# aalto-speech/AaltoASR

Measured on AMD Instinct MI355X. Metric: frames/sec GMM log-lik (39-d, 50k Gauss) + MFCC, 1/2/4/8 MI355X, higher is better.
Workload: dtype f32 (2-term fp16 split on the matrix cores, f32 accumulate); 1 GPU; configs[2]: full MFCC chain (FFT -> mel -> log -> DCT -> delta/delta-delta, CMS, normalisation) + 50000-Gaussian scoring + 2-byte LNA codes on 1 h of synthetic 16 kHz audio as 360 x 10 s utterances (449280 frames), int16 samples resident in HBM; dim=39, gaussians=50000, states=3125, gpus_flag=1

## Files before the change

aaltoasr_amd/csrc/lna_device.h:

```cpp
#pragma once
#include <hip/hip_runtime.h>

#include <cmath>
#include <cstdint>

namespace aasr {

#define LN2_D 0.69314718055994530942
#define LOG_TINY_D (-115.12925464970228420090)
#define LN_FLT_MIN_F (-87.33654475f)

__device__ __forceinline__ double float_cast_loglik(float ll) {
  if (ll >= LN_FLT_MIN_F) return (double)ll;
  if (ll < -103.98f) return -INFINITY;
  const float L1 = 1.44269502162933349609375f;
  const float L2 = 1.92596303350001e-08f;
  const float hi = ll * L1;
  const float lo = fmaf(ll, L1, -hi) + ll * L2;
  const float t = __builtin_amdgcn_exp2f(hi + 149.0f) * (1.0f + lo * 0.69314718f);
  const float q = rintf(t);
  if (q <= 0.0f) return -INFINITY;
  return (double)(__builtin_amdgcn_logf(q) * 0.69314718f) - 149.0 * LN2_D;
}

template <class T>
__device__ __forceinline__ T wave_reduce_max(T v) {
  for (int o = 32; o > 0; o >>= 1) {
    T u = __shfl_xor(v, o, 64);
    v = u > v ? u : v;
  }
  return v;
}
__device__ __forceinline__ double wave_reduce_sum(double v) {
  for (int o = 32; o > 0; o >>= 1) v += __shfl_xor(v, o, 64);
  return v;
}

__device__ __forceinline__ void lna_store(float lp, int lnabytes, int64_t o,
                                          float *__restrict__ lp_out,
                                          uint8_t *__restrict__ bytes_out) {
  if (lp_out) lp_out[o] = lp;
  if (bytes_out) {
    if (lnabytes == 4) {
      ((float *)bytes_out)[o] = lp;
    } else {
      unsigned short code;
      if (lp < -36.008f) {
        code = 0xffff;
      } else {
        int temp = (int)(-1820.0 * (double)lp + .5);
        unsigned b0 = (temp >> 8) & 255, b1 = temp & 255;
        code = (unsigned short)(b0 | (b1 << 8));
      }
      ((unsigned short *)bytes_out)[o] = code;
    }
  }
}

__device__ __forceinline__ float cast_f(float ll) {
  return ll >= LN_FLT_MIN_F ? ll : (float)float_cast_loglik(ll);
}


template <int VPT, int JSAFE = 0>
__device__ __forceinline__ void lna_row_from_registers(const float (&v)[VPT], int S, int tid, int wave, int lane,
                                                       double *red, int normalize, int lnabytes, int64_t f,
                                                       bool store, float *__restrict__ lp_out,
                                                       uint8_t *__restrict__ bytes_out) {
  double logz = 0.0;
  if (lnabytes == 2 && !lp_out) {
    float mr = -INFINITY;
#pragma unroll
    for (int j = 0; j < VPT; j++) mr = fmaxf(mr, v[j]);
    mr = wave_reduce_max(mr);
    if (lane == 0) red[wave] = (double)mr;
    __syncthreads();
    mr = (float)fmax(fmax(red[0], red[1]), fmax(red[2], red[3]));
    __syncthreads();
    if (mr >= -51.0f) {
      double z = 0.0;
      if (normalize) {
#pragma unroll
        for (int j = 0; j < VPT; j++) z += (double)__builtin_amdgcn_exp2f((v[j] - mr) * 1.44269504088896340736f);
      }
      z = wave_reduce_sum(z);
      if (lane == 0) red[4 + wave] = z;
      __syncthreads();
      z = (red[4] + red[5]) + (red[6] + red[7]);
      __syncthreads();
      if (normalize) logz = (double)mr + log(z);
      if (!store) return;
#pragma unroll
      for (int j = 0; j < VPT; j++) {
        const int i = tid + 256 * j;
        if (j < JSAFE || i < S) {
          const float lp = fmaxf((float)((double)v[j] - logz), (float)LOG_TINY_D);
          lna_store(lp, 2, f * (int64_t)S + i, nullptr, bytes_out);
        }
      }
      return;
    }
  }
  if (normalize) {
    float m = -INFINITY;
#pragma unroll
    for (int j = 0; j < VPT; j++) m = fmaxf(m, cast_f(v[j]));
    m = wave_reduce_max(m);
    if (lane == 0) red[wave] = (double)m;
    __syncthreads();
    m = (float)fmax(fmax(red[0], red[1]), fmax(red[2], red[3]));
    __syncthreads();
    double z = 0.0;
    if (m > -INFINITY) {
#pragma unroll
      for (int j = 0; j < VPT; j++)
        z += (double)__builtin_amdgcn_exp2f((cast_f(v[j]) - m) * 1.44269504088896340736f);
    }
    z = wave_reduce_sum(z);
    if (lane == 0) red[4 + wave] = z;
    __syncthreads();
    z = (red[4] + red[5]) + (red[6] + red[7]);
    __syncthreads();
    if (m > -INFINITY) logz = (double)m + log(z);
  }
  if (!store) return;
#pragma unroll
  for (int j = 0; j < VPT; j++) {
    const int i = tid + 256 * j;
    if (j < JSAFE || i < S) {
      const double vd = v[j] >= LN_FLT_MIN_F ? (double)v[j] : float_cast_loglik(v[j]);
      const float lp = fmaxf((float)(vd - logz), (float)LOG_TINY_D);
      lna_store(lp, lnabytes, f * (int64_t)S + i, lp_out, bytes_out);
    }
  }
}

}
```

aaltoasr_amd/csrc/lna_encode.hip:

```cpp
#include <hip/hip_runtime.h>

#include <algorithm>
#include <cmath>
#include <cstdlib>

#include "common.h"
#include "lna_device.h"

namespace aasr {

__global__ __launch_bounds__(256) void k_state_norm_lna(
    const float *__restrict__ loglik, int64_t F, int S, int64_t in_pitch, int normalize,
    int lnabytes, float *__restrict__ lp_out, uint8_t *__restrict__ bytes_out) {
  __shared__ double red[8];
  const int tid = threadIdx.x, wave = tid >> 6, lane = tid & 63;
  for (int64_t f = blockIdx.x; f < F; f += gridDim.x) {
    const float *row = loglik + f * in_pitch;
    double logz = 0.0;
    if (normalize) {
      double m = -INFINITY;
      for (int i = tid; i < S; i += 256) {
        double v = float_cast_loglik(row[i]);
        m = v > m ? v : m;
      }
      m = wave_reduce_max(m);
      if (lane == 0) red[wave] = m;
      __syncthreads();
      m = fmax(fmax(red[0], red[1]), fmax(red[2], red[3]));
      __syncthreads();
      if (m > -INFINITY) {
        double z = 0.0;
        for (int i = tid; i < S; i += 256) {
          double v = float_cast_loglik(row[i]);
          z += (double)expf((float)(v - m));
        }
        z = wave_reduce_sum(z);
        if (lane == 0) red[4 + wave] = z;
        __syncthreads();
        z = (red[4] + red[5]) + (red[6] + red[7]);
        __syncthreads();
        logz = m + log(z);
      }
    }
    for (int i = tid; i < S; i += 256) {
      double v = float_cast_loglik(row[i]);
      double lpd = v - logz;
      if (!(lpd >= LOG_TINY_D)) lpd = LOG_TINY_D;
      float lp = (float)lpd;
      int64_t o = f * (int64_t)S + i;
      if (lp_out) lp_out[o] = lp;
      if (bytes_out) {
        if (lnabytes == 4) {
          ((float *)bytes_out)[o] = lp;
        } else {
          unsigned short code;
          if ((double)lp < -36.008) {
            code = 0xffff;
          } else {
            int temp = (int)(-1820.0 * (double)lp + .5);
            unsigned b0 = (temp >> 8) & 255, b1 = temp & 255;
            code = (unsigned short)(b0 | (b1 << 8));
          }
          ((unsigned short *)bytes_out)[o] = code;
        }
      }
    }
  }
}


template <int VPT>
__global__ __launch_bounds__(256) void k_state_norm_lna_reg(
    const float *__restrict__ loglik, int64_t F, int S, int64_t in_pitch, int normalize, int lnabytes,
    float *__restrict__ lp_out, uint8_t *__restrict__ bytes_out, const int32_t *__restrict__ colmap) {
  __shared__ double red[8];
  const int tid = threadIdx.x, wave = tid >> 6, lane = tid & 63;
  constexpr int JSAFE = VPT == 4 ? 0 : VPT == 8 ? 4 : VPT == 10 ? 8 : VPT == 13 ? 10 : VPT == 16 ? 13 : 0;
  int col[VPT];
#pragma unroll
  for (int j = 0; j < VPT; j++) {
    const int i = tid + 256 * j;
    col[j] = (colmap && (j < JSAFE || i < S)) ? colmap[i] : i;
  }
  float vn[VPT];
  {
    const float *row = loglik + (int64_t)blockIdx.x * in_pitch;
#pragma unroll
    for (int j = 0; j < VPT; j++) {
      const int i = tid + 256 * j;
      vn[j] = ((j < JSAFE || i < S) && (int64_t)blockIdx.x < F) ? row[col[j]] : -INFINITY;
    }
  }
  for (int64_t f = blockIdx.x; f < F; f += gridDim.x) {
    float v[VPT];
#pragma unroll
    for (int j = 0; j < VPT; j++) v[j] = vn[j];
    if (f + gridDim.x < F) {
      const float *row = loglik + (f + gridDim.x) * in_pitch;
#pragma unroll
      for (int j = 0; j < VPT; j++) {
        const int i = tid + 256 * j;
        vn[j] = (j < JSAFE || i < S) ? row[col[j]] : -INFINITY;
      }
    }
    lna_row_from_registers<VPT, JSAFE>(v, S, tid, wave, lane, red, normalize, lnabytes, f, true, lp_out, bytes_out);
  }
}

__global__ __launch_bounds__(256) void k_state_norm_lna_f64(const double *__restrict__ lik, int64_t F, int S,
                                                            int normalize, int lnabytes, float *__restrict__ lp_out,
                                                            uint8_t *__restrict__ bytes_out) {
  __shared__ double red[4];
  const int tid = threadIdx.x, wave = tid >> 6, lane = tid & 63;
  for (int64_t f = blockIdx.x; f < F; f += gridDim.x) {
    const double *row = lik + f * (int64_t)S;
    double z = 1.0;
    if (normalize) {
      double part = 0.0;
      for (int i = tid; i < S; i += 256) part += (double)(float)row[i];
      part = wave_reduce_sum(part);
      __syncthreads();
      if (lane == 0) red[wave] = part;
      __syncthreads();
      z = (red[0] + red[1]) + (red[2] + red[3]);
      if (z == 0) z = 1.0;
    }
    for (int i = tid; i < S; i += 256) {
      const float o = (float)row[i];
      const double q = (double)o / z;
      const float lp = (float)(q < 1e-50 ? LOG_TINY_D : log(q));
      lna_store(lp, lnabytes, f * (int64_t)S + i, lp_out, bytes_out);
    }
  }
}

void lna_encode_f64_launch(const double *d_lik, int64_t F, int S, int normalize, int lnabytes, float *d_lp,
                           uint8_t *d_bytes, hipStream_t stream) {
  if (F <= 0 || S <= 0) return;
  const int64_t blocks = std::min<int64_t>(F, 8192);
  hipLaunchKernelGGL(k_state_norm_lna_f64, dim3((unsigned)blocks), dim3(256), 0, stream, d_lik, F, S, normalize, lnabytes,
                     d_lp, d_bytes);
  AASR_HIP(hipGetLastError());
}

void lna_encode_launch(const float *d_loglik, int64_t F, int S, int normalize,
                       int lnabytes, float *d_lp, uint8_t *d_bytes, hipStream_t stream, int64_t in_pitch,
                       const int32_t *d_colmap) {
  if (in_pitch <= 0) in_pitch = S;
  if (F <= 0 || S <= 0) return;
  if (d_colmap && S > 256 * 16) raise(AASR_ERR_UNSUPPORTED, "a column map needs the register-resident LNA kernels (S <= 4096)");
  int64_t blocks = F < (1 << 20) ? F : (1 << 20);
  int dev = 0, cus = 256;
  if (hipGetDevice(&dev) == hipSuccess) (void)hipDeviceGetAttribute(&cus, hipDeviceAttributeMultiprocessorCount, dev);
  if (S <= 256 * 16) blocks = std::min<int64_t>(blocks, (int64_t)cus * 32);
  if (S <= 256 * 4)
    hipLaunchKernelGGL(k_state_norm_lna_reg<4>, dim3((unsigned)blocks), dim3(256), 0, stream,
                       d_loglik, F, S, in_pitch, normalize, lnabytes, d_lp, d_bytes, d_colmap);
  else if (S <= 256 * 8)
    hipLaunchKernelGGL(k_state_norm_lna_reg<8>, dim3((unsigned)blocks), dim3(256), 0, stream,
                       d_loglik, F, S, in_pitch, normalize, lnabytes, d_lp, d_bytes, d_colmap);
  else if (S <= 256 * 10)
    hipLaunchKernelGGL(k_state_norm_lna_reg<10>, dim3((unsigned)blocks), dim3(256), 0, stream,
                       d_loglik, F, S, in_pitch, normalize, lnabytes, d_lp, d_bytes, d_colmap);
  else if (S <= 256 * 13)
    hipLaunchKernelGGL(k_state_norm_lna_reg<13>, dim3((unsigned)blocks), dim3(256), 0, stream,
                       d_loglik, F, S, in_pitch, normalize, lnabytes, d_lp, d_bytes, d_colmap);
  else if (S <= 256 * 16)
    hipLaunchKernelGGL(k_state_norm_lna_reg<16>, dim3((unsigned)blocks), dim3(256), 0, stream,
                       d_loglik, F, S, in_pitch, normalize, lnabytes, d_lp, d_bytes, d_colmap);
  else
    hipLaunchKernelGGL(k_state_norm_lna, dim3((unsigned)blocks), dim3(256), 0, stream, d_loglik,
                       F, S, in_pitch, normalize, lnabytes, d_lp, d_bytes);
  AASR_HIP(hipGetLastError());
}

}
```

Before: 43.12 million frames/s.

## Stage grouped LNA 2-byte codes in LDS and write them with wide nontemporal stores

Adds a grouped LNA encoding kernel that normalises G frames per block. It writes each frame's 2-byte codes into an LDS image and then copies the whole group to global memory with 8- or 16-byte nontemporal vector stores. The next row is prefetched with nontemporal loads while the current one is processed. The byte-swap for the code now uses a single perm instruction. The aim is to replace narrow 2-byte global stores with wide coalesced ones, at the cost of extra LDS use, which may lower occupancy, and an extra block-wide barrier per group.

```diff
diff --git a/aaltoasr_amd/csrc/lna_device.h b/aaltoasr_amd/csrc/lna_device.h
--- a/aaltoasr_amd/csrc/lna_device.h
+++ b/aaltoasr_amd/csrc/lna_device.h
@@ -36,6 +36,12 @@
   return v;
 }
 
+__device__ __forceinline__ unsigned lna_code16(float lp) {
+  const int temp = (int)(-1820.0 * (double)lp + .5);
+  const unsigned be = __builtin_amdgcn_perm(0u, (unsigned)temp, 0x0c0c0001u);
+  return lp < -36.008f ? 0xffffu : be;
+}
+
 __device__ __forceinline__ void lna_store(float lp, int lnabytes, int64_t o,
                                           float *__restrict__ lp_out,
                                           uint8_t *__restrict__ bytes_out) {
@@ -44,15 +50,7 @@
     if (lnabytes == 4) {
       ((float *)bytes_out)[o] = lp;
     } else {
-      unsigned short code;
-      if (lp < -36.008f) {
-        code = 0xffff;
-      } else {
-        int temp = (int)(-1820.0 * (double)lp + .5);
-        unsigned b0 = (temp >> 8) & 255, b1 = temp & 255;
-        code = (unsigned short)(b0 | (b1 << 8));
-      }
-      ((unsigned short *)bytes_out)[o] = code;
+      ((unsigned short *)bytes_out)[o] = (unsigned short)lna_code16(lp);
     }
   }
 }
@@ -66,7 +64,8 @@
 __device__ __forceinline__ void lna_row_from_registers(const float (&v)[VPT], int S, int tid, int wave, int lane,
                                                        double *red, int normalize, int lnabytes, int64_t f,
                                                        bool store, float *__restrict__ lp_out,
-                                                       uint8_t *__restrict__ bytes_out) {
+                                                       uint8_t *__restrict__ bytes_out,
+                                                       unsigned short *lds_row = nullptr) {
   double logz = 0.0;
   if (lnabytes == 2 && !lp_out) {
     float mr = -INFINITY;
@@ -95,7 +94,8 @@
         const int i = tid + 256 * j;
         if (j < JSAFE || i < S) {
           const float lp = fmaxf((float)((double)v[j] - logz), (float)LOG_TINY_D);
-          lna_store(lp, 2, f * (int64_t)S + i, nullptr, bytes_out);
+          if (lds_row) lds_row[i] = (unsigned short)lna_code16(lp);
+          else lna_store(lp, 2, f * (int64_t)S + i, nullptr, bytes_out);
         }
       }
       return;
@@ -130,7 +130,8 @@
     if (j < JSAFE || i < S) {
       const double vd = v[j] >= LN_FLT_MIN_F ? (double)v[j] : float_cast_loglik(v[j]);
       const float lp = fmaxf((float)(vd - logz), (float)LOG_TINY_D);
-      lna_store(lp, lnabytes, f * (int64_t)S + i, lp_out, bytes_out);
+      if (lds_row) lds_row[i] = (unsigned short)lna_code16(lp);
+      else lna_store(lp, lnabytes, f * (int64_t)S + i, lp_out, bytes_out);
     }
   }
 }
diff --git a/aaltoasr_amd/csrc/lna_encode.hip b/aaltoasr_amd/csrc/lna_encode.hip
--- a/aaltoasr_amd/csrc/lna_encode.hip
+++ b/aaltoasr_amd/csrc/lna_encode.hip
@@ -3,6 +3,7 @@
 #include <algorithm>
 #include <cmath>
 #include <cstdlib>
+#include <type_traits>
 
 #include "common.h"
 #include "lna_device.h"
@@ -107,6 +108,66 @@
   }
 }
 
+constexpr int kLnaRedBytes = 64;
+template <int VPT, int G>
+__global__ __launch_bounds__(256) void k_state_norm_lna_grp(
+    const float *__restrict__ loglik, int64_t F, int S, int64_t in_pitch, int normalize,
+    uint8_t *__restrict__ bytes_out, const int32_t *__restrict__ colmap) {
+  extern __shared__ __align__(16) unsigned char lna_smem[];
+  double *red = (double *)lna_smem;
+  unsigned char *img = lna_smem + kLnaRedBytes;
+  const int tid = threadIdx.x, wave = tid >> 6, lane = tid & 63;
+  constexpr int JSAFE = VPT == 4 ? 0 : VPT == 8 ? 4 : VPT == 10 ? 8 : VPT == 13 ? 10 : VPT == 16 ? 13 : 0;
+  int col[VPT];
+#pragma unroll
+  for (int j = 0; j < VPT; j++) {
+    const int i = tid + 256 * j;
+    col[j] = (colmap && (j < JSAFE || i < S)) ? colmap[i] : i;
+  }
+  typedef unsigned u32x4 __attribute__((ext_vector_type(4)));
+  typedef unsigned u32x2 __attribute__((ext_vector_type(2)));
+  using vec_t = typename std::conditional<G % 8 == 0, u32x4, u32x2>::type;
+  constexpr int W = (int)sizeof(vec_t);
+  static_assert(G % 4 == 0, "a group's codes must start on an 8-byte boundary at least");
+  const int64_t groups = (F + G - 1) / G;
+  float vn[VPT];
+  {
+    const int64_t f = (int64_t)blockIdx.x * G;
+    const float *row = loglik + f * in_pitch;
+#pragma unroll
+    for (int j = 0; j < VPT; j++) {
+      const int i = tid + 256 * j;
+      vn[j] = ((j < JSAFE || i < S) && f < F) ? row[col[j]] : -INFINITY;
+    }
+  }
+  for (int64_t grp = blockIdx.x; grp < groups; grp += gridDim.x) {
+    const int64_t f0 = grp * G;
+    const int nf = F - f0 < G ? (int)(F - f0) : G;
+    for (int g = 0; g < nf; g++) {
+      float v[VPT];
+#pragma unroll
+      for (int j = 0; j < VPT; j++) v[j] = vn[j];
+      const int64_t fnext = g + 1 < nf ? f0 + g + 1 : (grp + gridDim.x) * G;
+      if (fnext < F) {
+        const float *row = loglik + fnext * in_pitch;
+#pragma unroll
+        for (int j = 0; j < VPT; j++) {
+          const int i = tid + 256 * j;
+          vn[j] = (j < JSAFE || i < S) ? __builtin_nontemporal_load(&row[col[j]]) : -INFINITY;
+        }
+      }
+      lna_row_from_registers<VPT, JSAFE>(v, S, tid, wave, lane, red, normalize, 2, f0 + g, true, nullptr, nullptr,
+                                         (unsigned short *)img + g * S);
+    }
+    __syncthreads();
+    const int nbytes = nf * S * 2;
+    uint8_t *dst = bytes_out + f0 * (int64_t)S * 2;
+    for (int o = tid * W; o + W <= nbytes; o += 256 * W)
+      __builtin_nontemporal_store(*(const vec_t *)(img + o), (vec_t *)(dst + o));
+    for (int o = (nbytes & ~(W - 1)) + tid; o < nbytes; o += 256) dst[o] = img[o];
+  }
+}
+
 __global__ __launch_bounds__(256) void k_state_norm_lna_f64(const double *__restrict__ lik, int64_t F, int S,
                                                             int normalize, int lnabytes, float *__restrict__ lp_out,
                                                             uint8_t *__restrict__ bytes_out) {
@@ -141,6 +202,16 @@
   hipLaunchKernelGGL(k_state_norm_lna_f64, dim3((unsigned)blocks), dim3(256), 0, stream, d_lik, F, S, normalize, lnabytes,
                      d_lp, d_bytes);
   AASR_HIP(hipGetLastError());
+}
+
+#ifndef AASR_LNA_GROUP
+#define AASR_LNA_GROUP 4
+#endif
+constexpr int kLnaGroup = AASR_LNA_GROUP;
+constexpr int kLnaGroupBlocksPerCu = 32;
+constexpr size_t kLnaGroupLdsMax = 64 * 1024;
+static size_t lna_group_lds_bytes(int S) {
+  return (size_t)kLnaRedBytes + (((size_t)kLnaGroup * (size_t)S * 2 + 15) & ~(size_t)15);
 }
 
 void lna_encode_launch(const float *d_loglik, int64_t F, int S, int normalize,
@@ -153,6 +224,23 @@
   int dev = 0, cus = 256;
   if (hipGetDevice(&dev) == hipSuccess) (void)hipDeviceGetAttribute(&cus, hipDeviceAttributeMultiprocessorCount, dev);
   if (S <= 256 * 16) blocks = std::min<int64_t>(blocks, (int64_t)cus * 32);
+  if (lnabytes == 2 && !d_lp && d_bytes && S <= 256 * 16 && ((uintptr_t)d_bytes & 15) == 0 &&
+      lna_group_lds_bytes(S) <= kLnaGroupLdsMax) {
+    constexpr int G = kLnaGroup;
+    const int64_t groups = (F + G - 1) / G;
+    const unsigned gb = (unsigned)std::min<int64_t>(groups, (int64_t)cus * kLnaGroupBlocksPerCu);
+    const size_t lds = lna_group_lds_bytes(S);
+#define AASR_LNA_GRP(V) hipLaunchKernelGGL((k_state_norm_lna_grp<V, G>), dim3(gb), dim3(256), lds, stream, d_loglik, F, S, \
+                                           in_pitch, normalize, d_bytes, d_colmap)
+    if (S <= 256 * 4) AASR_LNA_GRP(4);
+    else if (S <= 256 * 8) AASR_LNA_GRP(8);
+    else if (S <= 256 * 10) AASR_LNA_GRP(10);
+    else if (S <= 256 * 13) AASR_LNA_GRP(13);
+    else AASR_LNA_GRP(16);
+#undef AASR_LNA_GRP
+    AASR_HIP(hipGetLastError());
+    return;
+  }
   if (S <= 256 * 4)
     hipLaunchKernelGGL(k_state_norm_lna_reg<4>, dim3((unsigned)blocks), dim3(256), 0, stream,
                        d_loglik, F, S, in_pitch, normalize, lnabytes, d_lp, d_bytes, d_colmap);
```

Measured after the change: 43.42 million frames/s (median of 6 runs). No clear change (+0.7%).
